# RishWijewardhena/vision-textile-inspection

Measured on AMD Instinct MI355X. Metric: frames/sec whole-node, YOLOv8n-seg 640x640 bs=64; mask IoU vs CPU ref, higher is better.
Workload: dtype f16x2

## Files before the change

### vision-textile-inspection_amd/csrc/conv.hip

```cpp
#include <algorithm>
#include <cstdlib>
#include <type_traits>

#include "conv_dev.h"

namespace vti {

__host__ __device__ inline int patch_dim(int t, int ks, int s, int mode) { return mode == 1 ? t : (t - 1) * s + ks; }

size_t stem_lds_bytes(int TH, int TW);

bool conv_wreg_ok(int ks, int stride, int mode, int WN, int NREP, int threads) {
    return mode == 0 && ks == 1 && stride == 1 && threads == 256 && WN == 4 && NREP <= 4;
}

size_t conv_lds_bytes(int ks, int stride, int mode, int TH, int TW, int WN, int NREP, int wreg) {
    if (mode == 1) return stem_lds_bytes(TH, TW);
    const int npix = patch_dim(TH, ks, stride, mode) * patch_dim(TW, ks, stride, mode);
    const size_t plane = (size_t)((npix + 15) & ~15) * 16;
    const int taps = mode == 1 ? 1 : ks * ks;
    size_t raw = 0;
    if (mode == 1) raw = (((size_t)(2 * TH + 1) * (2 * TW + 1) * 3) + 15) & ~(size_t)15;
    return 4 * plane + (wreg ? 0 : (size_t)WN * NREP * taps * 1024) + raw;
}

template <typename T, int KS, int S, int NREP, int WN, int NREP2 = 0, int NT = 256, bool WREG = false>
__global__ __launch_bounds__(NT, NT == 512 ? 1 : 2) void conv_kernel(const ConvParams p) {
    using vec = typename Tr<T>::vec;
    constexpr int VEC = Tr<T>::VEC, KC = Tr<T>::KC;
    constexpr int TAPS = KS * KS, PAD = KS / 2;
    constexpr int NTB = WN * NREP;
    constexpr int PP = NT / 4;
    constexpr int AR = NT == 512 ? 6 : (S == 2 ? 12 : 8);
    constexpr int BR = (NTB * TAPS * 64 + NT - 1) / NT;
    static_assert(!WREG || (KS == 1 && WN == NT / 64 && NREP2 == 0 && BR == NREP && NREP < 5), "WREG: one consumer wave per fragment");
    constexpr unsigned OOB = 0xFFFFFFFFu;
    extern __shared__ __attribute__((aligned(16))) char smem[];

    const int tid = threadIdx.x, lane = tid & 63, wave = tid >> 6;
    const int wn = wave % WN, wm = wave / WN;
    int t = blockIdx.x;
    const int tx = t % p.tiles_x; t /= p.tiles_x;
    const int ty = t % p.tiles_y;
// ... 16 lines not shown
        const bool v = pp < tile_px;
        const int pc = v ? pp : 0;
        const int py = (int)__umulhi((unsigned)pc, p.tw_magic), px = pc - py * p.TW;
        opy[m] = oy0 + py; opx[m] = ox0 + px;
        pvalid[m] = v && opy[m] < p.Hout && opx[m] < p.Wout;
        abase[m] = (lane >> 4) * plane_bytes + ((py * S) * PW + px * S) * 16;
    }

    f32x4 acc[MREP][NREP];
#pragma unroll
    for (int m = 0; m < MREP; ++m)
#pragma unroll
        for (int n = 0; n < NREP; ++n) acc[m][n] = (f32x4){0.f, 0.f, 0.f, 0.f};

    const size_t frame_elems = (size_t)p.Hin * p.Win * p.in_ld;
    const __amdgpu_buffer_rsrc_t rsA = __builtin_amdgcn_make_buffer_rsrc(
        (void*)((const T*)p.in + (size_t)b * frame_elems), 0, (int)(frame_elems * sizeof(T)), 0x00020000);
    const __amdgpu_buffer_rsrc_t rsB = __builtin_amdgcn_make_buffer_rsrc((void*)p.wpk, 0, (int)p.wpk_bytes, 0x00020000);

    const int iy0 = oy0 * S - PAD, ix0 = ox0 * S - PAD;
    const int q = (tid >> 3) & 3;
    const int pix0 = (tid >> 5) * 8 + (tid & 7);
    const int ldsA0 = q * plane_bytes + pix0 * 16;
    const int cvalid = (p.Cin - q * VEC + KC - 1) / KC;
    unsigned aoff[AR];
#pragma unroll
    for (int u = 0; u < AR; ++u) {
        const int pix = pix0 + PP * u;
        const int py = (int)__umulhi((unsigned)pix, p.pw_magic), px = pix - py * PW;
        const int y = iy0 + py, x = ix0 + px;
        const bool ok = pix < npix && (unsigned)y < (unsigned)p.Hin && (unsigned)x < (unsigned)p.Win;
        aoff[u] = ok ? (unsigned)(((y * p.Win + x) * p.in_ld + p.in_coff + q * VEC) * (int)sizeof(T)) : OOB;
    }
    constexpr bool BPRE = NREP < 5 || NT == 512;
    constexpr int PD = (KS == 1 && BPRE) ? 2 : 1;
    vec ra[PD][AR], rb[PD][BR];
    auto loadB = [&](int c, vec (&rbs)[BR]) {
        const unsigned sB = (unsigned)(((size_t)c * p.ntiles_n + nt0) * (TAPS * 1024));
#pragma unroll
        for (int u = 0; u < BR; ++u) {
            if constexpr (WREG) rbs[u] = buf_load16<vec>(rsB, (unsigned)((wn * NREP + u) * 64 + lane) * 16u, sB);
            else if (tid + u * NT < NTB * TAPS * 64) rbs[u] = buf_load16<vec>(rsB, (unsigned)(tid + u * NT) * 16u, sB);
        }
    };
    auto issue = [&](int c, vec (&ras)[AR], vec (&rbs)[BR]) {
        const bool qok = c < cvalid;
#pragma unroll
        for (int u = 0; u < AR; ++u)
            if (pix0 + PP * u < ((npix + 7) & ~7))
                ras[u] = buf_load16<vec>(rsA, qok ? aoff[u] : OOB, (unsigned)(c * KC * (int)sizeof(T)));
        if constexpr (BPRE) loadB(c, rbs);
    };
    auto commit = [&](int c, vec (&ras)[AR], vec (&rbs)[BR]) {
        if constexpr (!BPRE) loadB(c, rbs);
#pragma unroll
        for (int u = 0; u < AR; ++u)
            if (pix0 + PP * u < npix) *(vec*)(smA + ldsA0 + u * (PP * 16)) = ras[u];
        if constexpr (!WREG) {
#pragma unroll
            for (int u = 0; u < BR; ++u)
                if (tid + u * NT < NTB * TAPS * 64) *(vec*)(smB + (tid + u * NT) * 16) = rbs[u];
        }
    };
    auto chunk = [&](int c, auto set_c) {
        constexpr int SET = decltype(set_c)::value;
        if (c < 2) VTI_STAMP(1 + 5 * c);
        commit(c, ra[SET], rb[SET]);
// ... 31 lines not shown
#pragma unroll
            for (int s_ = 0; s_ < NSTEP; ++s_) {
                const int tp = s_ / MREP, mm = s_ % MREP;
                if (s_ + XD - 1 < NSTEP) xq[(s_ + XD - 1) % XD] = ldx(s_ + XD - 1);
                if (WD == 2 && mm == 0 && tp + 1 < TAPS) ldw(tp + 1, wq[(tp + 1) % WD]);
                __builtin_amdgcn_sched_barrier(0);
#pragma unroll
                for (int n = 0; n < NREP; ++n) acc[mm][n] = mma(wq[tp % WD][n], xq[s_ % XD], acc[mm][n]);
                __builtin_amdgcn_sched_barrier(0);
                if (WD == 1 && mm == MREP - 1 && tp + 1 < TAPS) ldw(tp + 1, wq[0]);
            }
            }
        }
        if (c < 2) VTI_STAMP(5 + 5 * c);
        if (c + 1 < p.nchunks) __syncthreads();
    };

    issue(0, ra[0], rb[0]);
    if constexpr (PD == 2) {
        if (p.nchunks > 1) issue(1, ra[1], rb[1]);
        for (int c = 0; c < p.nchunks; c += 2) {
            chunk(c, std::integral_constant<int, 0>{});
            if (c + 1 < p.nchunks) chunk(c + 1, std::integral_constant<int, 1>{});
        }
    } else {
        for (int c = 0; c < p.nchunks; ++c) chunk(c, std::integral_constant<int, 0>{});
    }

    VTI_STAMP(11);
    if constexpr (NREP2 == 0) {
        conv_epilogue<T, NREP>(p, acc, pvalid, opy, opx, b, nt0, wn, lane);
    } else {
        static_assert(WN == 1, "fused stage needs the whole Cout in one wave");
        conv_stage2<T, NREP, NREP2>(p, acc, pvalid, opy, opx, b, lane);
    }
    VTI_STAMP(12);
}

size_t convfold_lds_bytes(int TH, int TW) {
    const int npix = (TH + 2) * (TW + 2);
    return 4 * (size_t)((npix + 15) & ~15) * 16 + (size_t)16 * 4 * 1024;
}
bool convfold_supported(int c_in, int c_mid, int c_out, int ntiles2) {
    return c_in == c_mid && c_mid % 16 == 0 && c_out == 64 && c_in % 16 == 0 && c_in <= 64 && combo_has(FoldN2{}, ntiles2);
}

template <typename T, int NREP2, int NT = 256>
__global__ __launch_bounds__(NT, NT == 512 ? 1 : 2) void convfold_kernel(const ConvParams p) {
    using vec = typename Tr<T>::vec;
    constexpr int VEC = Tr<T>::VEC, KC = Tr<T>::KC;
    constexpr int NREP = 4, TAPS = 4, NTB = 16, AR = 8;
    constexpr int BR = NTB * TAPS * 64 / NT;
    constexpr int PPP = NT / 4;
    constexpr unsigned OOB = 0xFFFFFFFFu;
    extern __shared__ __attribute__((aligned(16))) char smem[];

    const int tid = threadIdx.x, lane = tid & 63, wave = (tid >> 6) & 3, mgrp = tid >> 8;
    const int py = wave >> 1, px = wave & 1;
    int t = blockIdx.x;
    const int tx = t % p.tiles_x; t /= p.tiles_x;
    const int ty = t % p.tiles_y;
    const int b = t / p.tiles_y;
    const int oy0 = ty * p.TH, ox0 = tx * p.TW;
    const int PH = p.TH + 2, PW = p.TW + 2;
    const int npix = PH * PW;
    const int plane_bytes = ((npix + 15) & ~15) * 16;
    char* smA = smem;
// ... 69 lines not shown
        {
            constexpr int NSTEP = TAPS * MREP;
            vec xq[3];
            vec wq[2][NREP];
            auto ldx = [&](int s_) -> vec {
                const int tp = s_ / MREP, mm = s_ % MREP;
                return *(const vec*)(smA + abase[mm] + ((tp >> 1) * PW + (tp & 1)) * 16);
            };
            auto ldw = [&](int tp, vec (&w)[NREP]) {
#pragma unroll
                for (int n = 0; n < NREP; ++n) w[n] = *(const vec*)(smB + ((wave * NREP + n) * TAPS + tp) * 1024 + lane * 16);
            };
            if constexpr (Tr<T>::H2) {
                auto ldw1 = [&](int tp, int n) -> vec { return *(const vec*)(smB + ((wave * NREP + n) * TAPS + tp) * 1024 + lane * 16); };
                h2_taps<NREP, MREP, TAPS, 3>(acc, ldx, ldw1);
            } else {
            ldw(0, wq[0]);
            xq[0] = ldx(0);
            xq[1] = ldx(1);
#pragma unroll
            for (int s_ = 0; s_ < NSTEP; ++s_) {
                const int tp = s_ / MREP, mm = s_ % MREP;
                if (s_ + 2 < NSTEP) xq[(s_ + 2) % 3] = ldx(s_ + 2);
                if (mm == 0 && tp + 1 < TAPS) ldw(tp + 1, wq[(tp + 1) % 2]);
                __builtin_amdgcn_sched_barrier(0);
#pragma unroll
                for (int n = 0; n < NREP; ++n) acc[mm][n] = mma(wq[tp % 2][n], xq[s_ % 3], acc[mm][n]);
                __builtin_amdgcn_sched_barrier(0);
            }
            }
        }
        if (c + 1 < p.nchunks) __syncthreads();
    }
    conv_stage2<T, NREP, NREP2, true>(p, acc, pvalid, opy, opx, b, lane);
}

hipError_t launch_convfold(int dtype, const ConvParams& p, size_t lds_bytes, hipStream_t st) {
    dim3 grid((unsigned)(p.B * p.tiles_y * p.tiles_x));
    if (grid.x == 0) return hipSuccess;
    const int nthr = p.nt == 512 ? 512 : 256;
    if (p.TH * p.TW > (nthr / 256) * MREP * 16 || ((p.TH + 2) * (p.TW + 2) + 7) / 8 * 32 > nthr * 8 || p.Cout != 256 || !p.out2 || !p.fold)
        return hipErrorInvalidValue;
    return with_conv_type(dtype, [&](auto t) -> hipError_t {
        using T = typename decltype(t)::type;
        if (p.nt == 512) {
            if constexpr (sizeof(T) == 4)
                return combo_dispatch(FoldN2{}, [&](auto c) {
                    return launch_lds<convfold_kernel<T, decltype(c)::v[0], 512>>(grid, dim3(512), lds_bytes, st, p);
                }, p.ntiles2);
            return hipErrorInvalidValue;
        }
        return combo_dispatch(FoldN2{}, [&](auto c) {
            return launch_lds<convfold_kernel<T, decltype(c)::v[0]>>(grid, dim3(256), lds_bytes, st, p);
        }, p.ntiles2);
    });
}

template <typename T, int NREP>
__global__ __launch_bounds__(256) void stem_kernel(const ConvParams p) {
    using vec = typename Tr<T>::vec;
    constexpr int VEC = Tr<T>::VEC, KC = Tr<T>::KC;
    constexpr int NCH = 32 / KC;
    extern __shared__ __attribute__((aligned(16))) char smem[];
    T* lut = (T*)smem;
    unsigned* raw32 = (unsigned*)(smem + 1024);
    const unsigned char* raw = (const unsigned char*)raw32;

// ... 300 lines not shown
        }
    }
    __syncthreads();
    VTI_STAMP(2);
    int opy[MREP], opx[MREP], sbase[MREP];
    bool pvalid[MREP];
#pragma unroll
    for (int m = 0; m < MREP; ++m) {
        const int pp = (wave * MREP + m) * 16 + (lane & 15);
        const int py = pp / SL_TW, px = pp - py * SL_TW;
        opy[m] = oy0 + py; opx[m] = ox0 + px;
        pvalid[m] = opy[m] < p.Hout && opx[m] < p.Wout;
        sbase[m] = ((2 * py) * SL_SW + 2 * px) * 16 * ES;
    }
    f32x4 acc[MREP][2];
#pragma unroll
    for (int m = 0; m < MREP; ++m) { acc[m][0] = (f32x4){0.f, 0.f, 0.f, 0.f}; acc[m][1] = (f32x4){0.f, 0.f, 0.f, 0.f}; }
#pragma unroll
    for (int s = 0; s < NS1; ++s) {
        const int tap = sizeof(T) == 2 ? 2 * s + (g >> 1) : s;
        const int tc = tap < 9 ? tap : 8;
        const int toff = ((tc / 3) * SL_SW + (tc % 3)) * 16 * ES + (sizeof(T) == 2 ? (g & 1) * 8 : g * 4) * ES;
        vec w1[2];
#pragma unroll
        for (int n = 0; n < 2; ++n) w1[n] = w1all[s][n];
#pragma unroll
        for (int m = 0; m < MREP; ++m) {
            const vec x = *(const vec*)(sout + sbase[m] + toff);
#pragma unroll
            for (int n = 0; n < 2; ++n) acc[m][n] = mma(w1[n], x, acc[m][n]);
        }
    }
    VTI_STAMP(3);
    if (p.out2) conv_stage2<T, 2, 2, false, true>(p, acc, pvalid, opy, opx, b, lane, &s2r);
    else conv_epilogue<T, 2>(p, acc, pvalid, opy, opx, b, 0, 0, lane);
    VTI_STAMP(12);
    }
}

void stem_l1_tile(int* th, int* tw) { *th = SL_TH; *tw = SL_TW; }

int stem_l1_grid(int dtype, int ntiles, bool persistent) {
    const int wgpc = (int)std::min<size_t>(2, (160 * 1024) / stem_l1_lds_bytes(dtype));
    if (!persistent) return ntiles;
    return std::min(ntiles, 256 * std::max(1, wgpc));
}

hipError_t launch_stem_l1(int dtype, const ConvParams& p, hipStream_t st, bool persistent) {
    dim3 grid((unsigned)stem_l1_grid(dtype, p.B * p.tiles_y * p.tiles_x, persistent));
    if (grid.x == 0) return hipSuccess;
    const size_t lds = stem_l1_lds_bytes(dtype);
    return with_conv_type(dtype, [&](auto t) { return launch_lds<stem_l1_kernel<typename decltype(t)::type>>(grid, dim3(256), lds, st, p); });
}

size_t stem_lds_bytes(int TH, int TW) { return 1024 + (size_t)(2 * TH + 1) * ((((2 * TW + 1) * 3 + 6) >> 2) * 4); }

using ConvTile3 = Combos<Ints<1, 1>, Ints<2, 1>, Ints<3, 1>, Ints<4, 1>, Ints<5, 1>, Ints<1, 2>, Ints<2, 2>, Ints<1, 4>>;
using ConvTile1 = decltype(concat(ConvTile3{}, Combos<Ints<3, 2>, Ints<4, 2>, Ints<5, 2>, Ints<2, 4>, Ints<3, 4>, Ints<4, 4>, Ints<5, 4>>{}));
using ConvTile1W = Combos<Ints<1, 4>, Ints<2, 4>, Ints<3, 4>, Ints<4, 4>>;
using StemNrep = Combos<Ints<1>, Ints<2>, Ints<3>, Ints<4>, Ints<5>>;

bool conv_cfg_fits(int ks, int stride, int mode, int TH, int TW, int WN, int NREP, int threads) {
    if (mode == 1) return WN == 1 && (2 * TH + 1) * (((2 * TW + 1) * 3 + 6) >> 2) < 65536;
    if (threads != 256 && !(threads == 512 && ks == 3 && stride == 1 && WN == 1)) return false;
    const int AR = threads == 512 ? 6 : (stride == 2 ? 12 : 8);
    const int npix = patch_dim(TH, ks, stride, mode) * patch_dim(TW, ks, stride, mode);
    if (((npix + 7) / 8) * 32 > threads * AR) return false;
// ... 20 lines not shown
static hipError_t launch_t(int ks, int stride, int nrep, int mode, const ConvParams& p, dim3 grid, size_t lds,
                           hipStream_t st) {
    if (p.ntiles2 > 0) {
        if (!(ks == 3 && stride == 1 && p.WN == 1 && mode == 0)) return hipErrorInvalidValue;
        return combo_dispatch(FusedPairs{}, [&](auto c) {
            using C = decltype(c);
            return p.nt == 512 ? launch_lds<conv_kernel<T, 3, 1, C::v[0], 1, C::v[1], 512>>(grid, dim3(512), lds, st, p)
                               : launch_lds<conv_kernel<T, 3, 1, C::v[0], 1, C::v[1]>>(grid, dim3(256), lds, st, p);
        }, nrep, p.ntiles2);
    }
    if (mode == 1)
        return combo_dispatch(StemNrep{}, [&](auto c) {
            hipLaunchKernelGGL((stem_kernel<T, decltype(c)::v[0]>), grid, dim3(256), lds, st, p);
            return hipGetLastError();
        }, nrep);
    if (ks == 1 && stride == 1) return launch_ks<T, 1, 1>(nrep, p, grid, lds, st);
    if (ks == 3 && stride == 1) return launch_ks<T, 3, 1>(nrep, p, grid, lds, st);
    if (ks == 3 && stride == 2) return launch_ks<T, 3, 2>(nrep, p, grid, lds, st);
    return hipErrorInvalidValue;
}

hipError_t launch_conv(int dtype, int ks, int stride, int nrep, int mode, const ConvParams& p, size_t lds_bytes,
                       hipStream_t st) {
    if (p.pk == 4) return launch_conv_pk2(dtype, nrep, p, lds_bytes, st);
    if (p.pk == 3) return launch_bneck_pk(dtype, nrep, p, lds_bytes, st);
    if (p.pk == 2) return launch_conv1_pk(dtype, nrep, p, lds_bytes, st);
    if (p.pk) return launch_conv_pk(dtype, nrep, p, lds_bytes, st);
    const int NTB = p.WN * nrep;
    dim3 grid((unsigned)(p.B * p.tiles_y * p.tiles_x), (unsigned)((p.ntiles_n + NTB - 1) / NTB));
    if (grid.x == 0) return hipSuccess;
    const int nwaves = p.nt == 512 ? 8 : 4;
    if (p.wreg && !conv_wreg_ok(ks, stride, mode, p.WN, nrep, p.nt)) return hipErrorInvalidValue;
    lds_bytes = std::max(lds_bytes, conv_lds_bytes(ks, stride, mode, p.TH, p.TW, p.WN, nrep, p.wreg));
    if ((p.nt != 256 && p.nt != 512) || (p.nt == 512 && p.ntiles2 == 0)) return hipErrorInvalidValue;
    if (p.TH * p.TW > (nwaves / p.WN) * MREP * 16 || (p.WN != 1 && p.WN != 2 && p.WN != 4)) return hipErrorInvalidValue;
    return with_conv_type(dtype, [&](auto t) { return launch_t<typename decltype(t)::type>(ks, stride, nrep, mode, p, grid, lds_bytes, st); });
}

}
```

### vision-textile-inspection_amd/csrc/conv_dev.h

```cpp
#pragma once
#include "vti_internal.h"

namespace vti {

typedef _Float16 half_t;
typedef _Float16 half8 __attribute__((ext_vector_type(8)));
typedef _Float16 half4 __attribute__((ext_vector_type(4)));
typedef float f32x4 __attribute__((ext_vector_type(4)));

typedef unsigned u32x4 __attribute__((ext_vector_type(4)));

struct h2_t { unsigned u; };
struct h2x4 { u32x4 u; };
constexpr float H2_SX = 16.0f;

template <typename T> struct Tr;
template <> struct Tr<half_t> { typedef half8 vec; static constexpr int VEC = 8, KC = 32; static constexpr bool H16 = true, F32 = false, H2 = false; };
template <> struct Tr<float> { typedef f32x4 vec; static constexpr int VEC = 4, KC = 16; static constexpr bool H16 = false, F32 = true, H2 = false; };
template <> struct Tr<h2_t> { typedef h2x4 vec; static constexpr int VEC = 4, KC = 16; static constexpr bool H16 = false, F32 = false, H2 = true; };

typedef _Float16 half2v __attribute__((ext_vector_type(2)));
__device__ __forceinline__ unsigned h2_enc(float v) {
    half2v p;
    p[0] = (half_t)__builtin_fmaf(v, H2_SX, 0.0f);
// ... 341 lines not shown
    }
}

template <typename V> __device__ __forceinline__ V buf_load16(__amdgpu_buffer_rsrc_t r, unsigned voff, unsigned soff) {
    const u32x4 v = __builtin_amdgcn_raw_buffer_load_b128(r, voff, soff, 0);
    return __builtin_bit_cast(V, v);
}

template <typename T, int NREP, int NREP2> struct Stage2Regs {
    using vec = typename Tr<T>::vec;
    static constexpr int KT = sizeof(T) == 2 ? (NREP + 1) / 2 : NREP;
    vec w2[KT][NREP2];
    f32x4 bias1[NREP];
    f32x4 bias2[NREP2];
};

template <typename T, int NREP, int NREP2>
__device__ __forceinline__ void stage2_preload(const ConvParams& p, int lane, bool fold, Stage2Regs<T, NREP, NREP2>& r) {
    using vec = typename Tr<T>::vec;
    const __amdgpu_buffer_rsrc_t rsW2 = __builtin_amdgcn_make_buffer_rsrc(
        (void*)p.w2, 0, (int)(Stage2Regs<T, NREP, NREP2>::KT * p.ntiles2 * 1024), 0x00020000);
#pragma unroll
    for (int t2 = 0; t2 < Stage2Regs<T, NREP, NREP2>::KT; ++t2)
#pragma unroll
        for (int n = 0; n < NREP2; ++n) r.w2[t2][n] = buf_load16<vec>(rsW2, (unsigned)(((t2 * p.ntiles2 + n) * 64 + lane) * 16), 0u);
    const float* b1 = p.bias + (fold ? 4 * (16 * NREP) : 0) + (lane >> 4) * 4 * NREP;
#pragma unroll
    for (int n = 0; n < NREP; ++n) r.bias1[n] = *(const f32x4*)(b1 + 4 * n);
    const int crun2 = p.nat2 ? (lane >> 4) * 4 : (lane >> 4) * 4 * NREP2, cstep2 = p.nat2 ? 16 : 4;
#pragma unroll
    for (int n = 0; n < NREP2; ++n) r.bias2[n] = *(const f32x4*)(p.bias2 + crun2 + cstep2 * n);
}

template <typename T, int NREP, int NREP2, bool FOLD = false, bool PRE = false>
__device__ __forceinline__ void conv_stage2(const ConvParams& p, f32x4 (&acc)[MREP][NREP], const bool (&pvalid)[MREP],
                                            const int (&opy)[MREP], const int (&opx)[MREP], int b, int lane,
                                            const Stage2Regs<T, NREP, NREP2>* pre = nullptr, bool interior = false) {
    const int OW = FOLD ? 2 * p.Wout : p.Wout;
    using vec = typename Tr<T>::vec;
    constexpr bool FAST = !Tr<T>::F32;
    constexpr int KT = sizeof(T) == 2 ? (NREP + 1) / 2 : NREP;
    const __amdgpu_buffer_rsrc_t rsW2 = __builtin_amdgcn_make_buffer_rsrc(
        (void*)p.w2, 0, (int)(KT * p.ntiles2 * 1024), 0x00020000);
    f32x4 bias1[FOLD ? MREP : 1][NREP];
    if (PRE && (!FOLD || interior)) {
#pragma unroll
        for (int m = 0; m < (FOLD ? MREP : 1); ++m)
#pragma unroll
            for (int n = 0; n < NREP; ++n) bias1[m][n] = pre->bias1[n];
    } else if constexpr (FOLD) {
#pragma unroll
        for (int m = 0; m < MREP; ++m) {
            const int cy = opy[m] == 0 ? 0 : (opy[m] == 2 * p.Hout - 1 ? 2 : 1), cx = opx[m] == 0 ? 0 : (opx[m] == OW - 1 ? 2 : 1);
            const float* bt = p.bias + (cy * 3 + cx) * (16 * NREP) + (lane >> 4) * 4 * NREP;
#pragma unroll
            for (int n = 0; n < NREP; ++n) bias1[m][n] = *(const f32x4*)(bt + 4 * n);
        }
    } else {
#pragma unroll
        for (int n = 0; n < NREP; ++n) bias1[0][n] = *(const f32x4*)(p.bias + (lane >> 4) * 4 * NREP + 4 * n);
    }
    f32x4 acc2[MREP][NREP2];
#pragma unroll
    for (int m = 0; m < MREP; ++m)
#pragma unroll
        for (int n = 0; n < NREP2; ++n) acc2[m][n] = (f32x4){0.f, 0.f, 0.f, 0.f};
#pragma unroll
    for (int t2 = 0; t2 < KT; ++t2) {
        vec w2[NREP2];
#pragma unroll
        for (int n = 0; n < NREP2; ++n) {
            if constexpr (PRE) w2[n] = pre->w2[t2][n];
            else w2[n] = buf_load16<vec>(rsW2, (unsigned)(((t2 * p.ntiles2 + n) * 64 + lane) * 16), 0u);
        }
#pragma unroll
        for (int m = 0; m < MREP; ++m) {
            vec x;
            if constexpr (sizeof(T) == 2) {
#pragma unroll
                for (int h = 0; h < 2; ++h) {
                    const int n1 = 2 * t2 + h;
                    f32x4 v = {0.f, 0.f, 0.f, 0.f};
                    if (n1 < NREP) {
                        v = acc_bias<T>(acc[m][n1 < NREP ? n1 : 0], bias1[FOLD ? m : 0][n1 < NREP ? n1 : 0], p.alpha);
                        if (p.act) v = silu4<FAST>(v);
                    }
#pragma unroll
                    for (int j = 0; j < 4; ++j) x[h * 4 + j] = (T)v[j];
                }
            } else {
                f32x4 v = acc_bias<T>(acc[m][t2], bias1[FOLD ? m : 0][t2], p.alpha);
                if (p.act) v = silu4<FAST>(v);
                if constexpr (Tr<T>::H2) x.u = pack4<T>(v);
                else {
#pragma unroll
                    for (int j = 0; j < 4; ++j) x[j] = v[j];
                }
            }
#pragma unroll
            for (int n = 0; n < NREP2; ++n) acc2[m][n] = mma(w2[n], x, acc2[m][n]);
        }
    }
    [[maybe_unused]] const int tid = threadIdx.x;
    VTI_STAMP(13);
    f32x4 bias2[NREP2];
    const int crun2 = p.nat2 ? (lane >> 4) * 4 : (lane >> 4) * 4 * NREP2;
    const int cstep2 = p.nat2 ? 16 : 4;
#pragma unroll
    for (int n = 0; n < NREP2; ++n) {
        if constexpr (PRE) bias2[n] = pre->bias2[n];
        else bias2[n] = *(const f32x4*)(p.bias2 + crun2 + cstep2 * n);
    }
    if constexpr (NREP2 == 4) {
        if (p.act2 == 3) {
            const int g = lane >> 4;
#pragma unroll
            for (int m = 0; m < MREP; ++m) {
                float d4[4];
#pragma unroll
                for (int n = 0; n < 4; ++n) {
                    const f32x4 v = acc_bias<T>(acc2[m][n], bias2[n], p.alpha2);
                    float mx = fmaxf(fmaxf(v[0], v[1]), fmaxf(v[2], v[3]));
                    mx = fmaxf(mx, __shfl_xor(mx, 16));
                    mx = fmaxf(mx, __shfl_xor(mx, 32));
                    float e[4];
#pragma unroll
                    for (int j = 0; j < 4; ++j) {
                        if constexpr (FAST) e[j] = __builtin_amdgcn_exp2f((v[j] - mx) * 1.4426950408889634f);
                        else e[j] = expf(v[j] - mx);
                    }
                    float s = (e[0] + e[1]) + (e[2] + e[3]);
                    float w = (e[0] * (float)(4 * g) + e[1] * (float)(4 * g + 1)) + (e[2] * (float)(4 * g + 2) + e[3] * (float)(4 * g + 3));
                    s += __shfl_xor(s, 16); w += __shfl_xor(w, 16);
                    s += __shfl_xor(s, 32); w += __shfl_xor(w, 32);
                    d4[n] = w / s;
                }
                const float ax = (float)opx[m] + 0.5f, ay = (float)opy[m] + 0.5f;
                const float x1 = ax - d4[0], y1 = ay - d4[1], x2 = ax + d4[2], y2 = ay + d4[3];
                const float comp = g == 0 ? ((x1 + x2) / 2.0f) * p.dfl_stride : g == 1 ? ((y1 + y2) / 2.0f) * p.dfl_stride
                                 : g == 2 ? (x2 - x1) * p.dfl_stride : (y2 - y1) * p.dfl_stride;
                if (pvalid[m])
                    ((float*)p.out2)[((size_t)b * p.out2_bstride + (size_t)opy[m] * OW + opx[m]) * p.out2_ld + p.out2_coff + g] = comp;
            }
            return;
        }
    }
    if constexpr (sizeof(T) == 2 && NREP2 % 2 == 0) {
        if (!p.nat2 && !p.out2_f32 && !p.scalar_store2 && (p.Cout2 & 7) == 0 && ((p.out2_ld | p.out2_coff) & 7) == 0) {
#pragma unroll
            for (int m = 0; m < MREP; ++m) {
                if (!pvalid[m]) continue;
                half_t* op = (half_t*)p.out2 + ((size_t)b * p.out2_bstride + (size_t)opy[m] * OW + opx[m]) * p.out2_ld + p.out2_coff + crun2;
#pragma unroll
                for (int n = 0; n < NREP2; n += 2) {
                    if (crun2 + 4 * n >= p.Cout2) continue;
                    f32x4 v0 = acc_bias<T>(acc2[m][n], bias2[n], p.alpha2), v1 = acc_bias<T>(acc2[m][n + 1], bias2[n + 1], p.alpha2);
                    if (p.act2 == 1) { v0 = silu4<FAST>(v0); v1 = silu4<FAST>(v1); }
                    half8 hv;
#pragma unroll
                    for (int j = 0; j < 4; ++j) { hv[j] = (half_t)v0[j]; hv[4 + j] = (half_t)v1[j]; }
                    *(half8*)(op + 4 * n) = hv;
                }
            }
            return;
        }
    }
    const bool want_best = p.act2 == 2 && p.best != nullptr;
#pragma unroll
    for (int m = 0; m < MREP; ++m) {
        const size_t pix = (size_t)b * p.out2_bstride + (size_t)opy[m] * OW + opx[m];
        const size_t o0 = pix * p.out2_ld + p.out2_coff;
        float bv = -INFINITY;
        int bc = 0x7fffffff;
        if (!want_best && !pvalid[m]) continue;
#pragma unroll
        for (int n = 0; n < NREP2; ++n) {
            const int cout0 = crun2 + cstep2 * n;
            if (cout0 >= p.Cout2) continue;
            f32x4 v = acc_bias<T>(acc2[m][n], bias2[n], p.alpha2);
            if (p.act2 == 1) v = silu4<FAST>(v);
            else if (p.act2 == 2) {
#pragma unroll
                for (int j = 0; j < 4; ++j) {
                    if constexpr (FAST) v[j] = __builtin_amdgcn_rcpf(1.0f + __builtin_amdgcn_exp2f(v[j] * -1.4426950408889634f));
                    else v[j] = 1.0f / (1.0f + expf(-v[j]));
                }
                if (want_best) {
                    if ((p.Cout2 & 3) == 0) {
#pragma unroll
                        for (int j = 0; j < 4; ++j)
                            if (v[j] > bv) { bv = v[j]; bc = cout0 + j; }
                    } else {
#pragma unroll
                        for (int j = 0; j < 4; ++j)
                            if (cout0 + j < p.Cout2 && v[j] > bv) { bv = v[j]; bc = cout0 + j; }
                    }
                }
            }
            if (!pvalid[m]) continue;
            const size_t o = o0 + cout0;
            if (p.scalar_store2) {
#pragma unroll
                for (int j = 0; j < 4; ++j) {
                    if (cout0 + j < p.Cout2) {
                        if (p.out2_f32) ((float*)p.out2)[o + j] = v[j];
                        else if constexpr (Tr<T>::H2) ((unsigned*)p.out2)[o + j] = h2_enc(v[j]);
                        else ((T*)p.out2)[o + j] = (T)v[j];
                    }
                }
            } else if (p.out2_f32 || Tr<T>::F32) {
                *(f32x4*)((float*)p.out2 + o) = v;
            } else if constexpr (Tr<T>::H2) {
                *(u32x4*)((unsigned*)p.out2 + o) = pack4<T>(v);
            } else {
                half4 hv;
#pragma unroll
                for (int j = 0; j < 4; ++j) hv[j] = (half_t)v[j];
                *(half4*)((half_t*)p.out2 + o) = hv;
            }
        }
        if (want_best) {
#pragma unroll
            for (int o = 16; o <= 32; o <<= 1) {
                const float ob = __shfl_xor(bv, o);
                const int oc = __shfl_xor(bc, o);
                if (ob > bv || (ob == bv && oc < bc)) { bv = ob; bc = oc; }
            }
            if (lane < 16 && pvalid[m]) *(float2*)(p.best + pix * 2) = make_float2(bv, (float)(bc == 0x7fffffff ? 0 : bc));
        }
    }
}

template <int... V> struct Ints { static constexpr int v[] = {V...}; };
template <typename... C> struct Combos {};
template <typename... A, typename... B> Combos<A..., B...> concat(Combos<A...>, Combos<B...>) { return {}; }

template <int... V, typename... K> constexpr bool ints_eq(Ints<V...>, K... key) { return ((V == key) && ...); }
template <typename... C, typename... K> constexpr bool combo_has(Combos<C...>, K... key) { return (... || ints_eq(C{}, key...)); }
template <typename... C, typename F, typename... K> hipError_t combo_dispatch(Combos<C...>, F&& f, K... key) {
    hipError_t e = hipErrorInvalidValue;
    (void)(... || (ints_eq(C{}, key...) && (e = f(C{}), true)));
    return e;
}

using FusedPairs = Combos<Ints<2, 2>, Ints<3, 2>, Ints<4, 1>, Ints<4, 2>, Ints<4, 4>, Ints<4, 5>, Ints<5, 5>>;
using FoldN2 = Combos<Ints<1>, Ints<2>, Ints<4>>;

template <typename T> struct Type { using type = T; };
template <typename F> hipError_t with_conv_type(int dtype, F&& f) {
    if (dtype == VTI_F16) return f(Type<half_t>{});
    if (dtype == VTI_H2) return f(Type<h2_t>{});
    return f(Type<float>{});
}

}
```

### vision-textile-inspection_amd/csrc/conv_pk.hip

```cpp
#include <algorithm>
#include <cstdlib>
#include <type_traits>

#include "conv_dev.h"

namespace vti {

constexpr int PK_PWP = 24;
constexpr int PK_TW = 20;
constexpr int PK_ROWS = 4;
constexpr int PK_MAXD = 9;
constexpr int PK_MAXD2 = 13;

using ConvPkS1 = Combos<Ints<1, 1>, Ints<2, 1>, Ints<3, 1>, Ints<4, 1>, Ints<5, 1>, Ints<1, 2>, Ints<2, 2>, Ints<3, 2>, Ints<4, 2>, Ints<1, 4>,
                        Ints<2, 4>>;
using ConvPkS2 = Combos<Ints<1, 4>, Ints<2, 2>, Ints<4, 1>, Ints<2, 1>, Ints<1, 2>>;
using Conv1Pk = decltype(concat(ConvPkS1{}, Combos<Ints<4, 4>>{}));
bool conv_pk_instantiated(int nrep, int wn) { return combo_has(ConvPkS1{}, nrep, wn); }
bool conv_pk2_instantiated(int nrep, int wn) { return combo_has(ConvPkS2{}, nrep, wn); }
bool conv1_pk_instantiated(int nrep, int wn) { return combo_has(Conv1Pk{}, nrep, wn); }
using Conv1PkWH2 = Combos<Ints<2, 2, 4>, Ints<2, 2, 6>, Ints<2, 2, 8>, Ints<2, 2, 12>, Ints<2, 2, 16>,
                          Ints<2, 4, 4>, Ints<2, 4, 6>, Ints<2, 4, 8>, Ints<2, 4, 12>, Ints<2, 4, 16>>;
using Conv1PkWF16 = Combos<Ints<2, 2, 2>, Ints<2, 2, 3>, Ints<2, 2, 4>, Ints<2, 2, 6>, Ints<2, 2, 8>,
                           Ints<2, 4, 2>, Ints<2, 4, 3>, Ints<2, 4, 4>, Ints<2, 4, 6>, Ints<2, 4, 8>, Ints<4, 1, 2>>;
// ... 324 lines not shown
                    }
                } else if constexpr (sizeof(T) == 2) {
                    typedef unsigned u32x2 __attribute__((ext_vector_type(2)));
#pragma unroll
                    for (int n = 0; n < NREP; ++n) {
                        half4 hv;
#pragma unroll
                        for (int j = 0; j < 4; ++j) hv[j] = (half_t)v[n][j];
                        const bool cv = pv && crun + 4 * n < p.Cout;
                        __builtin_amdgcn_raw_buffer_store_b64(__builtin_bit_cast(u32x2, hv), rsO, cv ? ob + n * 8 : OOB, 0u, 0);
                    }
                } else {
#pragma unroll
                    for (int n = 0; n < NREP; ++n) {
                        const bool cv = pv && crun + 4 * n < p.Cout;
                        __builtin_amdgcn_raw_buffer_store_b128(pack4<T>(v[n]), rsO, cv ? ob + n * 16 : OOB, 0u, 0);
                    }
                }
            }
            };
            if (p.has_res) epi(std::true_type{}); else epi(std::false_type{});
        } else {
            int opy[MREP], opx[MREP];
            bool pvalid[MREP];
#pragma unroll
            for (int m = 0; m < MREP; ++m) {
                opy[m] = oy0 + ry[m]; opx[m] = ox0 + rx[m];
                pvalid[m] = opy[m] < p.Hout && opx[m] < p.Wout;
            }
            if constexpr (FOLD) {
#pragma unroll
                for (int m = 0; m < MREP; ++m) { opy[m] = 2 * opy[m] + fpy; opx[m] = 2 * opx[m] + fpx; }
                const bool interior = oy0 > 0 && oy0 + p.TH < p.Hout && ox0 > 0 && ox0 + PK_TW < p.Wout;
                conv_stage2<T, NREP, NREP2, true, true>(p, acc, pvalid, opy, opx, b, lane, &s2r, interior);
            } else if constexpr (NREP2 == 0) conv_epilogue<T, NREP>(p, acc, pvalid, opy, opx, b, nt0, wn, lane);
            else conv_stage2<T, NREP, NREP2>(p, acc, pvalid, opy, opx, b, lane);
        }
        VTI_STAMP(12);
        const int tn = t + tstride;
        if (tn >= tend) break;
        t = tn;
        tile_coords(t, b, oy0, ox0);
    }
}


constexpr int PK1_MAXP = 5;

size_t conv1_pk_lds_bytes(int nwm, int WN, int NREP, int nchunks, int depth, int wstat, int cps) {
    const size_t stage = (size_t)nwm * 80 * 64 * cps;
    const size_t wch = (size_t)WN * NREP * 1024;
    const size_t wbytes = wstat == 2 ? 0 : wstat ? (size_t)nchunks * wch : (size_t)depth * wch * cps;
    return (size_t)depth * stage + wbytes + 1024  + (size_t)WN * NREP * 64;
}

template <typename V> __device__ __forceinline__ void reg_touch(V& v) {
    if constexpr (std::is_same<V, h2x4>::value) asm volatile("" : "+v"(v.u));
    else asm volatile("" : "+v"(v));
}

template <typename T, int NREP, int WN, int CPS, int NCH = 0>
__global__ __launch_bounds__(512) void conv1_pk(const ConvParams p) {
    using vec = typename Tr<T>::vec;
    constexpr int VEC = Tr<T>::VEC, KC = Tr<T>::KC, ES = (int)sizeof(T);
    constexpr int NTB = WN * NREP;
    constexpr int WCH = NTB * 1024;
    constexpr unsigned OOB = 0x80000000u;
    constexpr bool FAST = !Tr<T>::F32;
    extern __shared__ __attribute__((aligned(16))) char smem[];
// ... 880 lines not shown
```

Measured before the change: 16830.

## Stage fused 1x1 second-stage weights in LDS and block stage2 over pixel groups

In the fused conv kernels, the second-stage 1x1 weights are loaded cooperatively into LDS once per block. For the h2 type they are pre-split into hi/lo half fragments, so each MMA uses two f16 MFMAs without unpacking per use. The stage2 loop is now templated on a weight source (LDS, registers or memory) and processes pixel rows in blocks of MB. This cuts register pressure and lets weight loads be double-buffered. The B-prefetch is disabled for the h2 NREP=4 fused case. The cost is extra LDS, two block barriers, and per-pixel store code that has been split out into a helper.

```diff
diff --git a/vision-textile-inspection_amd/csrc/conv.hip b/vision-textile-inspection_amd/csrc/conv.hip
--- a/vision-textile-inspection_amd/csrc/conv.hip
+++ b/vision-textile-inspection_amd/csrc/conv.hip
@@ -9,6 +9,8 @@
 __host__ __device__ inline int patch_dim(int t, int ks, int s, int mode) { return mode == 1 ? t : (t - 1) * s + ks; }
 
 size_t stem_lds_bytes(int TH, int TW);
+
+template <typename T, int NREP> constexpr int s2_mb() { return Tr<T>::H2 && NREP == 4 ? 1 : 2; }
 
 bool conv_wreg_ok(int ks, int stride, int mode, int WN, int NREP, int threads) {
     return mode == 0 && ks == 1 && stride == 1 && threads == 256 && WN == 4 && NREP <= 4;
@@ -91,7 +93,7 @@
         const bool ok = pix < npix && (unsigned)y < (unsigned)p.Hin && (unsigned)x < (unsigned)p.Win;
         aoff[u] = ok ? (unsigned)(((y * p.Win + x) * p.in_ld + p.in_coff + q * VEC) * (int)sizeof(T)) : OOB;
     }
-    constexpr bool BPRE = NREP < 5 || NT == 512;
+    constexpr bool BPRE = (NREP < 5 && !(Tr<T>::H2 && NREP == 4 && NREP2 > 0 && NT == 256)) || NT == 512;
     constexpr int PD = (KS == 1 && BPRE) ? 2 : 1;
     vec ra[PD][AR], rb[PD][BR];
     auto loadB = [&](int c, vec (&rbs)[BR]) {
@@ -189,7 +191,8 @@
         conv_epilogue<T, NREP>(p, acc, pvalid, opy, opx, b, nt0, wn, lane);
     } else {
         static_assert(WN == 1, "fused stage needs the whole Cout in one wave");
-        conv_stage2<T, NREP, NREP2>(p, acc, pvalid, opy, opx, b, lane);
+        stage2_to_lds<T, NREP, NREP2, NT>(p, smem, tid);
+        conv_stage2<T, NREP, NREP2, false, false, s2_mb<T, NREP>()>(p, acc, pvalid, opy, opx, b, lane, W2Lds<T, NREP2>{smem + lane * 16});
     }
     VTI_STAMP(12);
 }
@@ -325,7 +328,13 @@
         }
         if (c + 1 < p.nchunks) __syncthreads();
     }
-    conv_stage2<T, NREP, NREP2, true>(p, acc, pvalid, opy, opx, b, lane);
+    if constexpr (NREP2 >= 4) {
+        static_assert(stage2_lds_bytes((int)sizeof(T), Tr<T>::H2, NREP, NREP2) <= (size_t)NTB * TAPS * 1024, "the staged 1x1 fragments overlay the weight planes");
+        stage2_to_lds<T, NREP, NREP2, NT>(p, smem, tid);
+        conv_stage2<T, NREP, NREP2, true, false, 2>(p, acc, pvalid, opy, opx, b, lane, W2Lds<T, NREP2>{smem + lane * 16});
+    } else {
+        conv_stage2<T, NREP, NREP2, true, false, MREP>(p, acc, pvalid, opy, opx, b, lane, w2_mem<T>(p, stage2_kt((int)sizeof(T), NREP), lane));
+    }
 }
 
 hipError_t launch_convfold(int dtype, const ConvParams& p, size_t lds_bytes, hipStream_t st) {
@@ -692,7 +701,7 @@
         }
     }
     VTI_STAMP(3);
-    if (p.out2) conv_stage2<T, 2, 2, false, true>(p, acc, pvalid, opy, opx, b, lane, &s2r);
+    if (p.out2) conv_stage2<T, 2, 2, false, true, 1>(p, acc, pvalid, opy, opx, b, lane, W2Regs<T, 2, 2>{&s2r}, &s2r);
     else conv_epilogue<T, 2>(p, acc, pvalid, opy, opx, b, 0, 0, lane);
     VTI_STAMP(12);
     }
@@ -779,6 +788,7 @@
     const int nwaves = p.nt == 512 ? 8 : 4;
     if (p.wreg && !conv_wreg_ok(ks, stride, mode, p.WN, nrep, p.nt)) return hipErrorInvalidValue;
     lds_bytes = std::max(lds_bytes, conv_lds_bytes(ks, stride, mode, p.TH, p.TW, p.WN, nrep, p.wreg));
+    if (p.ntiles2 > 0) lds_bytes = std::max(lds_bytes, stage2_lds_bytes(dtype == VTI_F16 ? 2 : 4, dtype == VTI_H2, nrep, p.ntiles2));
     if ((p.nt != 256 && p.nt != 512) || (p.nt == 512 && p.ntiles2 == 0)) return hipErrorInvalidValue;
     if (p.TH * p.TW > (nwaves / p.WN) * MREP * 16 || (p.WN != 1 && p.WN != 2 && p.WN != 4)) return hipErrorInvalidValue;
     return with_conv_type(dtype, [&](auto t) { return launch_t<typename decltype(t)::type>(ks, stride, nrep, mode, p, grid, lds_bytes, st); });
diff --git a/vision-textile-inspection_amd/csrc/conv_dev.h b/vision-textile-inspection_amd/csrc/conv_dev.h
--- a/vision-textile-inspection_amd/csrc/conv_dev.h
+++ b/vision-textile-inspection_amd/csrc/conv_dev.h
@@ -397,16 +397,199 @@
     for (int n = 0; n < NREP2; ++n) r.bias2[n] = *(const f32x4*)(p.bias2 + crun2 + cstep2 * n);
 }
 
-template <typename T, int NREP, int NREP2, bool FOLD = false, bool PRE = false>
+struct h2prep { u32x4 wh, wl; };
+__device__ __forceinline__ f32x4 mma(h2prep w, h2x4 x, f32x4 c) {
+    const half8 xv = __builtin_bit_cast(half8, x.u);
+    c = __builtin_amdgcn_mfma_f32_16x16x32_f16(__builtin_bit_cast(half8, w.wh), xv, c, 0, 0, 0);
+    c = __builtin_amdgcn_mfma_f32_16x16x32_f16(__builtin_bit_cast(half8, w.wl), xv, c, 0, 0, 0);
+    return c;
+}
+constexpr int stage2_kt(int es, int nrep) { return es == 2 ? (nrep + 1) / 2 : nrep; }
+constexpr size_t stage2_lds_bytes(int es, bool h2, int nrep, int nrep2) { return (size_t)stage2_kt(es, nrep) * nrep2 * (h2 ? 2048 : 1024); }
+
+template <typename T, int NREP, int NREP2, int NT>
+__device__ __forceinline__ void stage2_to_lds(const ConvParams& p, char* smem, int tid) {
+    using vec = typename Tr<T>::vec;
+    constexpr int KT = stage2_kt((int)sizeof(T), NREP), NF = KT * NREP2, NP = (NF * 64 + NT - 1) / NT;
+    const __amdgpu_buffer_rsrc_t rsW2 = __builtin_amdgcn_make_buffer_rsrc((void*)p.w2, 0, (int)(KT * p.ntiles2 * 1024), 0x00020000);
+    vec r[NP];
+#pragma unroll
+    for (int u = 0; u < NP; ++u) {
+        const int i = tid + u * NT, f = i >> 6;
+        if (i < NF * 64) r[u] = buf_load16<vec>(rsW2, (unsigned)((((f / NREP2) * p.ntiles2 + f % NREP2) * 64 + (i & 63)) * 16), 0u);
+    }
+    __syncthreads();
+#pragma unroll
+    for (int u = 0; u < NP; ++u) {
+        const int i = tid + u * NT;
+        if (i >= NF * 64) continue;
+        if constexpr (Tr<T>::H2) {
+            u32x4 wh, wl;
+#pragma unroll
+            for (int j = 0; j < 4; ++j) { wh[j] = __builtin_amdgcn_perm(r[u].u[j], r[u].u[j], 0x01000100u); wl[j] = r[u].u[j] >> 16; }
+            char* d = smem + (i >> 6) * 2048 + (i & 63) * 16;
+            *(u32x4*)d = wh;
+            *(u32x4*)(d + 1024) = wl;
+        } else {
+            *(vec*)(smem + i * 16) = r[u];
+        }
+    }
+    __syncthreads();
+}
+template <typename T, int NREP2> struct W2Lds {
+    static constexpr bool ROW = false;
+    const char* base;
+    __device__ __forceinline__ auto operator()(int t2, int n) const {
+        if constexpr (Tr<T>::H2) {
+            const char* f = base + (t2 * NREP2 + n) * 2048;
+            return h2prep{*(const u32x4*)f, *(const u32x4*)(f + 1024)};
+        } else {
+            return *(const typename Tr<T>::vec*)(base + (t2 * NREP2 + n) * 1024);
+        }
+    }
+};
+template <typename T, int NREP, int NREP2> struct W2Regs {
+    static constexpr bool ROW = false;
+    const Stage2Regs<T, NREP, NREP2>* r;
+    __device__ __forceinline__ typename Tr<T>::vec operator()(int t2, int n) const { return r->w2[t2][n]; }
+};
+template <typename T> struct W2Mem {
+    static constexpr bool ROW = true;
+    __amdgpu_buffer_rsrc_t rs;
+    int ntiles2, lane;
+    __device__ __forceinline__ typename Tr<T>::vec operator()(int t2, int n) const {
+        return buf_load16<typename Tr<T>::vec>(rs, (unsigned)(((t2 * ntiles2 + n) * 64 + lane) * 16), 0u);
+    }
+};
+template <typename T> __device__ __forceinline__ W2Mem<T> w2_mem(const ConvParams& p, int kt, int lane) {
+    return W2Mem<T>{__builtin_amdgcn_make_buffer_rsrc((void*)p.w2, 0, (int)(kt * p.ntiles2 * 1024), 0x00020000), p.ntiles2, lane};
+}
+
+template <typename T, int NREP2>
+__device__ __forceinline__ void stage2_store(const ConvParams& p, const f32x4 (&acc2)[NREP2], const f32x4 (&bias2)[NREP2], bool pvalid,
+                                             int opy, int opx, int b, int lane, int OW) {
+    constexpr bool FAST = !Tr<T>::F32;
+    const int crun2 = p.nat2 ? (lane >> 4) * 4 : (lane >> 4) * 4 * NREP2;
+    const int cstep2 = p.nat2 ? 16 : 4;
+    if constexpr (NREP2 == 4) {
+        if (p.act2 == 3) {
+            const int g = lane >> 4;
+            float d4[4];
+#pragma unroll
+            for (int n = 0; n < 4; ++n) {
+                const f32x4 v = acc_bias<T>(acc2[n], bias2[n], p.alpha2);
+                float mx = fmaxf(fmaxf(v[0], v[1]), fmaxf(v[2], v[3]));
+                mx = fmaxf(mx, __shfl_xor(mx, 16));
+                mx = fmaxf(mx, __shfl_xor(mx, 32));
+                float e[4];
+#pragma unroll
+                for (int j = 0; j < 4; ++j) {
+                    if constexpr (FAST) e[j] = __builtin_amdgcn_exp2f((v[j] - mx) * 1.4426950408889634f);
+                    else e[j] = expf(v[j] - mx);
+                }
+                float s = (e[0] + e[1]) + (e[2] + e[3]);
+                float w = (e[0] * (float)(4 * g) + e[1] * (float)(4 * g + 1)) + (e[2] * (float)(4 * g + 2) + e[3] * (float)(4 * g + 3));
+                s += __shfl_xor(s, 16); w += __shfl_xor(w, 16);
+                s += __shfl_xor(s, 32); w += __shfl_xor(w, 32);
+                d4[n] = w / s;
+            }
+            const float ax = (float)opx + 0.5f, ay = (float)opy + 0.5f;
+            const float x1 = ax - d4[0], y1 = ay - d4[1], x2 = ax + d4[2], y2 = ay + d4[3];
+            const float comp = g == 0 ? ((x1 + x2) / 2.0f) * p.dfl_stride : g == 1 ? ((y1 + y2) / 2.0f) * p.dfl_stride
+                             : g == 2 ? (x2 - x1) * p.dfl_stride : (y2 - y1) * p.dfl_stride;
+            if (pvalid)
+                ((float*)p.out2)[((size_t)b * p.out2_bstride + (size_t)opy * OW + opx) * p.out2_ld + p.out2_coff + g] = comp;
+            return;
+        }
+    }
+    if constexpr (sizeof(T) == 2 && NREP2 % 2 == 0) {
+        if (!p.nat2 && !p.out2_f32 && !p.scalar_store2 && (p.Cout2 & 7) == 0 && ((p.out2_ld | p.out2_coff) & 7) == 0) {
+            if (!pvalid) return;
+            half_t* op = (half_t*)p.out2 + ((size_t)b * p.out2_bstride + (size_t)opy * OW + opx) * p.out2_ld + p.out2_coff + crun2;
+#pragma unroll
+            for (int n = 0; n < NREP2; n += 2) {
+                if (crun2 + 4 * n >= p.Cout2) continue;
+                f32x4 v0 = acc_bias<T>(acc2[n], bias2[n], p.alpha2), v1 = acc_bias<T>(acc2[n + 1], bias2[n + 1], p.alpha2);
+                if (p.act2 == 1) { v0 = silu4<FAST>(v0); v1 = silu4<FAST>(v1); }
+                half8 hv;
+#pragma unroll
+                for (int j = 0; j < 4; ++j) { hv[j] = (half_t)v0[j]; hv[4 + j] = (half_t)v1[j]; }
+                *(half8*)(op + 4 * n) = hv;
+            }
+            return;
+        }
+    }
+    const bool want_best = p.act2 == 2 && p.best != nullptr;
+    const size_t pix = (size_t)b * p.out2_bstride + (size_t)opy * OW + opx;
+    const size_t o0 = pix * p.out2_ld + p.out2_coff;
+    float bv = -INFINITY;
+    int bc = 0x7fffffff;
+    if (!want_best && !pvalid) return;
+#pragma unroll
+    for (int n = 0; n < NREP2; ++n) {
+        const int cout0 = crun2 + cstep2 * n;
+        if (cout0 >= p.Cout2) continue;
+        f32x4 v = acc_bias<T>(acc2[n], bias2[n], p.alpha2);
+        if (p.act2 == 1) v = silu4<FAST>(v);
+        else if (p.act2 == 2) {
+#pragma unroll
+            for (int j = 0; j < 4; ++j) {
+                if constexpr (FAST) v[j] = __builtin_amdgcn_rcpf(1.0f + __builtin_amdgcn_exp2f(v[j] * -1.4426950408889634f));
+                else v[j] = 1.0f / (1.0f + expf(-v[j]));
+            }
+            if (want_best) {
+                if ((p.Cout2 & 3) == 0) {
+#pragma unroll
+                    for (int j = 0; j < 4; ++j)
+                        if (v[j] > bv) { bv = v[j]; bc = cout0 + j; }
+                } else {
+#pragma unroll
+                    for (int j = 0; j < 4; ++j)
+                        if (cout0 + j < p.Cout2 && v[j] > bv) { bv = v[j]; bc = cout0 + j; }
+                }
+            }
+        }
+        if (!pvalid) continue;
+        const size_t o = o0 + cout0;
+        if (p.scalar_store2) {
+#pragma unroll
+            for (int j = 0; j < 4; ++j) {
+                if (cout0 + j < p.Cout2) {
+                    if (p.out2_f32) ((float*)p.out2)[o + j] = v[j];
+                    else if constexpr (Tr<T>::H2) ((unsigned*)p.out2)[o + j] = h2_enc(v[j]);
+                    else ((T*)p.out2)[o + j] = (T)v[j];
+                }
+            }
+        } else if (p.out2_f32 || Tr<T>::F32) {
+            *(f32x4*)((float*)p.out2 + o) = v;
+        } else if constexpr (Tr<T>::H2) {
+            *(u32x4*)((unsigned*)p.out2 + o) = pack4<T>(v);
+        } else {
+            half4 hv;
+#pragma unroll
+            for (int j = 0; j < 4; ++j) hv[j] = (half_t)v[j];
+            *(half4*)((half_t*)p.out2 + o) = hv;
+        }
+    }
+    if (want_best) {
+#pragma unroll
+        for (int o = 16; o <= 32; o <<= 1) {
+            const float ob = __shfl_xor(bv, o);
+            const int oc = __shfl_xor(bc, o);
+            if (ob > bv || (ob == bv && oc < bc)) { bv = ob; bc = oc; }
+        }
+        if (lane < 16 && pvalid) *(float2*)(p.best + pix * 2) = make_float2(bv, (float)(bc == 0x7fffffff ? 0 : bc));
+    }
+}
+
+template <typename T, int NREP, int NREP2, bool FOLD, bool PRE, int MB, class SRC>
 __device__ __forceinline__ void conv_stage2(const ConvParams& p, f32x4 (&acc)[MREP][NREP], const bool (&pvalid)[MREP],
-                                            const int (&opy)[MREP], const int (&opx)[MREP], int b, int lane,
+                                            const int (&opy)[MREP], const int (&opx)[MREP], int b, int lane, SRC w2src,
                                             const Stage2Regs<T, NREP, NREP2>* pre = nullptr, bool interior = false) {
     const int OW = FOLD ? 2 * p.Wout : p.Wout;
     using vec = typename Tr<T>::vec;
     constexpr bool FAST = !Tr<T>::F32;
-    constexpr int KT = sizeof(T) == 2 ? (NREP + 1) / 2 : NREP;
-    const __amdgpu_buffer_rsrc_t rsW2 = __builtin_amdgcn_make_buffer_rsrc(
-        (void*)p.w2, 0, (int)(KT * p.ntiles2 * 1024), 0x00020000);
+    constexpr int KT = stage2_kt((int)sizeof(T), NREP), NU = KT * NREP2;
     f32x4 bias1[FOLD ? MREP : 1][NREP];
     if (PRE && (!FOLD || interior)) {
 #pragma unroll
@@ -425,174 +608,80 @@
 #pragma unroll
         for (int n = 0; n < NREP; ++n) bias1[0][n] = *(const f32x4*)(p.bias + (lane >> 4) * 4 * NREP + 4 * n);
     }
-    f32x4 acc2[MREP][NREP2];
-#pragma unroll
-    for (int m = 0; m < MREP; ++m)
-#pragma unroll
-        for (int n = 0; n < NREP2; ++n) acc2[m][n] = (f32x4){0.f, 0.f, 0.f, 0.f};
-#pragma unroll
-    for (int t2 = 0; t2 < KT; ++t2) {
-        vec w2[NREP2];
-#pragma unroll
-        for (int n = 0; n < NREP2; ++n) {
-            if constexpr (PRE) w2[n] = pre->w2[t2][n];
-            else w2[n] = buf_load16<vec>(rsW2, (unsigned)(((t2 * p.ntiles2 + n) * 64 + lane) * 16), 0u);
-        }
-#pragma unroll
-        for (int m = 0; m < MREP; ++m) {
-            vec x;
-            if constexpr (sizeof(T) == 2) {
-#pragma unroll
-                for (int h = 0; h < 2; ++h) {
-                    const int n1 = 2 * t2 + h;
-                    f32x4 v = {0.f, 0.f, 0.f, 0.f};
-                    if (n1 < NREP) {
-                        v = acc_bias<T>(acc[m][n1 < NREP ? n1 : 0], bias1[FOLD ? m : 0][n1 < NREP ? n1 : 0], p.alpha);
-                        if (p.act) v = silu4<FAST>(v);
-                    }
-#pragma unroll
-                    for (int j = 0; j < 4; ++j) x[h * 4 + j] = (T)v[j];
+    auto build_x = [&](int m, int t2) -> vec {
+        vec x;
+        if constexpr (sizeof(T) == 2) {
+#pragma unroll
+            for (int h = 0; h < 2; ++h) {
+                const int n1 = 2 * t2 + h;
+                f32x4 v = {0.f, 0.f, 0.f, 0.f};
+                if (n1 < NREP) {
+                    v = acc_bias<T>(acc[m][n1 < NREP ? n1 : 0], bias1[FOLD ? m : 0][n1 < NREP ? n1 : 0], p.alpha);
+                    if (p.act) v = silu4<FAST>(v);
+                }
+#pragma unroll
+                for (int j = 0; j < 4; ++j) x[h * 4 + j] = (T)v[j];
+            }
+        } else {
+            f32x4 v = acc_bias<T>(acc[m][t2], bias1[FOLD ? m : 0][t2], p.alpha);
+            if (p.act) v = silu4<FAST>(v);
+            if constexpr (Tr<T>::H2) x.u = pack4<T>(v);
+            else {
+#pragma unroll
+                for (int j = 0; j < 4; ++j) x[j] = v[j];
+            }
+        }
+        return x;
+    };
+#pragma unroll
+    for (int m0 = 0; m0 < MREP; m0 += MB) {
+        if (m0 > 0) asm volatile("" ::: "memory");
+        f32x4 acc2[MB][NREP2];
+#pragma unroll
+        for (int i = 0; i < MB; ++i)
+#pragma unroll
+            for (int n = 0; n < NREP2; ++n) acc2[i][n] = (f32x4){0.f, 0.f, 0.f, 0.f};
+        decltype(w2src(0, 0)) wq[SRC::ROW ? NREP2 : 2];
+        if constexpr (!SRC::ROW) wq[0] = w2src(0, 0);
+#pragma unroll
+        for (int t2 = 0; t2 < KT; ++t2) {
+            if constexpr (SRC::ROW) {
+#pragma unroll
+                for (int n = 0; n < NREP2; ++n) wq[n] = w2src(t2, n);
+#pragma unroll
+                for (int i = 0; i < MB; ++i) {
+                    if (m0 + i >= MREP) continue;
+                    const vec x = build_x(m0 + i, t2);
+#pragma unroll
+                    for (int n = 0; n < NREP2; ++n) acc2[i][n] = mma(wq[n], x, acc2[i][n]);
                 }
             } else {
-                f32x4 v = acc_bias<T>(acc[m][t2], bias1[FOLD ? m : 0][t2], p.alpha);
-                if (p.act) v = silu4<FAST>(v);
-                if constexpr (Tr<T>::H2) x.u = pack4<T>(v);
-                else {
-#pragma unroll
-                    for (int j = 0; j < 4; ++j) x[j] = v[j];
-                }
-            }
-#pragma unroll
-            for (int n = 0; n < NREP2; ++n) acc2[m][n] = mma(w2[n], x, acc2[m][n]);
-        }
-    }
-    [[maybe_unused]] const int tid = threadIdx.x;
-    VTI_STAMP(13);
-    f32x4 bias2[NREP2];
-    const int crun2 = p.nat2 ? (lane >> 4) * 4 : (lane >> 4) * 4 * NREP2;
-    const int cstep2 = p.nat2 ? 16 : 4;
-#pragma unroll
-    for (int n = 0; n < NREP2; ++n) {
-        if constexpr (PRE) bias2[n] = pre->bias2[n];
-        else bias2[n] = *(const f32x4*)(p.bias2 + crun2 + cstep2 * n);
-    }
-    if constexpr (NREP2 == 4) {
-        if (p.act2 == 3) {
-            const int g = lane >> 4;
-#pragma unroll
-            for (int m = 0; m < MREP; ++m) {
-                float d4[4];
-#pragma unroll
-                for (int n = 0; n < 4; ++n) {
-                    const f32x4 v = acc_bias<T>(acc2[m][n], bias2[n], p.alpha2);
-                    float mx = fmaxf(fmaxf(v[0], v[1]), fmaxf(v[2], v[3]));
-                    mx = fmaxf(mx, __shfl_xor(mx, 16));
-                    mx = fmaxf(mx, __shfl_xor(mx, 32));
-                    float e[4];
-#pragma unroll
-                    for (int j = 0; j < 4; ++j) {
-                        if constexpr (FAST) e[j] = __builtin_amdgcn_exp2f((v[j] - mx) * 1.4426950408889634f);
-                        else e[j] = expf(v[j] - mx);
-                    }
-                    float s = (e[0] + e[1]) + (e[2] + e[3]);
-                    float w = (e[0] * (float)(4 * g) + e[1] * (float)(4 * g + 1)) + (e[2] * (float)(4 * g + 2) + e[3] * (float)(4 * g + 3));
-                    s += __shfl_xor(s, 16); w += __shfl_xor(w, 16);
-                    s += __shfl_xor(s, 32); w += __shfl_xor(w, 32);
-                    d4[n] = w / s;
-                }
-                const float ax = (float)opx[m] + 0.5f, ay = (float)opy[m] + 0.5f;
-                const float x1 = ax - d4[0], y1 = ay - d4[1], x2 = ax + d4[2], y2 = ay + d4[3];
-                const float comp = g == 0 ? ((x1 + x2) / 2.0f) * p.dfl_stride : g == 1 ? ((y1 + y2) / 2.0f) * p.dfl_stride
-                                 : g == 2 ? (x2 - x1) * p.dfl_stride : (y2 - y1) * p.dfl_stride;
-                if (pvalid[m])
-                    ((float*)p.out2)[((size_t)b * p.out2_bstride + (size_t)opy[m] * OW + opx[m]) * p.out2_ld + p.out2_coff + g] = comp;
-            }
-            return;
-        }
-    }
-    if constexpr (sizeof(T) == 2 && NREP2 % 2 == 0) {
-        if (!p.nat2 && !p.out2_f32 && !p.scalar_store2 && (p.Cout2 & 7) == 0 && ((p.out2_ld | p.out2_coff) & 7) == 0) {
-#pragma unroll
-            for (int m = 0; m < MREP; ++m) {
-                if (!pvalid[m]) continue;
-                half_t* op = (half_t*)p.out2 + ((size_t)b * p.out2_bstride + (size_t)opy[m] * OW + opx[m]) * p.out2_ld + p.out2_coff + crun2;
-#pragma unroll
-                for (int n = 0; n < NREP2; n += 2) {
-                    if (crun2 + 4 * n >= p.Cout2) continue;
-                    f32x4 v0 = acc_bias<T>(acc2[m][n], bias2[n], p.alpha2), v1 = acc_bias<T>(acc2[m][n + 1], bias2[n + 1], p.alpha2);
-                    if (p.act2 == 1) { v0 = silu4<FAST>(v0); v1 = silu4<FAST>(v1); }
-                    half8 hv;
-#pragma unroll
-                    for (int j = 0; j < 4; ++j) { hv[j] = (half_t)v0[j]; hv[4 + j] = (half_t)v1[j]; }
-                    *(half8*)(op + 4 * n) = hv;
-                }
-            }
-            return;
-        }
-    }
-    const bool want_best = p.act2 == 2 && p.best != nullptr;
-#pragma unroll
-    for (int m = 0; m < MREP; ++m) {
-        const size_t pix = (size_t)b * p.out2_bstride + (size_t)opy[m] * OW + opx[m];
-        const size_t o0 = pix * p.out2_ld + p.out2_coff;
-        float bv = -INFINITY;
-        int bc = 0x7fffffff;
-        if (!want_best && !pvalid[m]) continue;
-#pragma unroll
-        for (int n = 0; n < NREP2; ++n) {
-            const int cout0 = crun2 + cstep2 * n;
-            if (cout0 >= p.Cout2) continue;
-            f32x4 v = acc_bias<T>(acc2[m][n], bias2[n], p.alpha2);
-            if (p.act2 == 1) v = silu4<FAST>(v);
-            else if (p.act2 == 2) {
-#pragma unroll
-                for (int j = 0; j < 4; ++j) {
-                    if constexpr (FAST) v[j] = __builtin_amdgcn_rcpf(1.0f + __builtin_amdgcn_exp2f(v[j] * -1.4426950408889634f));
-                    else v[j] = 1.0f / (1.0f + expf(-v[j]));
-                }
-                if (want_best) {
-                    if ((p.Cout2 & 3) == 0) {
-#pragma unroll
-                        for (int j = 0; j < 4; ++j)
-                            if (v[j] > bv) { bv = v[j]; bc = cout0 + j; }
-                    } else {
-#pragma unroll
-                        for (int j = 0; j < 4; ++j)
-                            if (cout0 + j < p.Cout2 && v[j] > bv) { bv = v[j]; bc = cout0 + j; }
-                    }
-                }
-            }
-            if (!pvalid[m]) continue;
-            const size_t o = o0 + cout0;
-            if (p.scalar_store2) {
-#pragma unroll
-                for (int j = 0; j < 4; ++j) {
-                    if (cout0 + j < p.Cout2) {
-                        if (p.out2_f32) ((float*)p.out2)[o + j] = v[j];
-                        else if constexpr (Tr<T>::H2) ((unsigned*)p.out2)[o + j] = h2_enc(v[j]);
-                        else ((T*)p.out2)[o + j] = (T)v[j];
-                    }
-                }
-            } else if (p.out2_f32 || Tr<T>::F32) {
-                *(f32x4*)((float*)p.out2 + o) = v;
-            } else if constexpr (Tr<T>::H2) {
-                *(u32x4*)((unsigned*)p.out2 + o) = pack4<T>(v);
-            } else {
-                half4 hv;
-#pragma unroll
-                for (int j = 0; j < 4; ++j) hv[j] = (half_t)v[j];
-                *(half4*)((half_t*)p.out2 + o) = hv;
-            }
-        }
-        if (want_best) {
-#pragma unroll
-            for (int o = 16; o <= 32; o <<= 1) {
-                const float ob = __shfl_xor(bv, o);
-                const int oc = __shfl_xor(bc, o);
-                if (ob > bv || (ob == bv && oc < bc)) { bv = ob; bc = oc; }
-            }
-            if (lane < 16 && pvalid[m]) *(float2*)(p.best + pix * 2) = make_float2(bv, (float)(bc == 0x7fffffff ? 0 : bc));
-        }
+                vec x[MB];
+#pragma unroll
+                for (int i = 0; i < MB; ++i)
+                    if (m0 + i < MREP) x[i] = build_x(m0 + i, t2);
+#pragma unroll
+                for (int n = 0; n < NREP2; ++n) {
+                    const int u = t2 * NREP2 + n;
+                    if (u + 1 < NU) wq[(u + 1) & 1] = w2src((u + 1) / NREP2, (u + 1) % NREP2);
+#pragma unroll
+                    for (int i = 0; i < MB; ++i)
+                        if (m0 + i < MREP) acc2[i][n] = mma(wq[u & 1], x[i], acc2[i][n]);
+                }
+            }
+        }
+        f32x4 bias2[NREP2];
+        {
+            const int crun2 = p.nat2 ? (lane >> 4) * 4 : (lane >> 4) * 4 * NREP2, cstep2 = p.nat2 ? 16 : 4;
+#pragma unroll
+            for (int n = 0; n < NREP2; ++n) {
+                if constexpr (PRE) bias2[n] = pre->bias2[n];
+                else bias2[n] = *(const f32x4*)(p.bias2 + crun2 + cstep2 * n);
+            }
+        }
+#pragma unroll
+        for (int i = 0; i < MB; ++i)
+            if (m0 + i < MREP) stage2_store<T, NREP2>(p, acc2[i], bias2, pvalid[m0 + i], opy[m0 + i], opx[m0 + i], b, lane, OW);
     }
 }
 
diff --git a/vision-textile-inspection_amd/csrc/conv_pk.hip b/vision-textile-inspection_amd/csrc/conv_pk.hip
--- a/vision-textile-inspection_amd/csrc/conv_pk.hip
+++ b/vision-textile-inspection_amd/csrc/conv_pk.hip
@@ -380,9 +380,9 @@
 #pragma unroll
                 for (int m = 0; m < MREP; ++m) { opy[m] = 2 * opy[m] + fpy; opx[m] = 2 * opx[m] + fpx; }
                 const bool interior = oy0 > 0 && oy0 + p.TH < p.Hout && ox0 > 0 && ox0 + PK_TW < p.Wout;
-                conv_stage2<T, NREP, NREP2, true, true>(p, acc, pvalid, opy, opx, b, lane, &s2r, interior);
+                conv_stage2<T, NREP, NREP2, true, true, 1>(p, acc, pvalid, opy, opx, b, lane, W2Regs<T, NREP, NREP2>{&s2r}, &s2r, interior);
             } else if constexpr (NREP2 == 0) conv_epilogue<T, NREP>(p, acc, pvalid, opy, opx, b, nt0, wn, lane);
-            else conv_stage2<T, NREP, NREP2>(p, acc, pvalid, opy, opx, b, lane);
+            else conv_stage2<T, NREP, NREP2, false, false, MREP>(p, acc, pvalid, opy, opx, b, lane, w2_mem<T>(p, stage2_kt(ES, NREP), lane));
         }
         VTI_STAMP(12);
         const int tn = t + tstride;
```

Result: no change. 16870, median of 6 (+0.2%).
